# invictus717/MiCo

Measured on AMD Instinct MI355X. Metric: omni-modal samples/sec (ViT-g/14 fwd+bwd), higher is better.
Workload: dtype fp16

## Files before the change

### include/mico_hip.h

```cpp
#ifndef MICO_HIP_H
#define MICO_HIP_H
#include <stdint.h>

#ifdef __cplusplus
extern "C" {
#endif

#define MICO_F16 0
#define MICO_BF16 1
#define MICO_F32 2

#define MICO_OK 0
#define MICO_EINVAL (-22)
#define MICO_ELAUNCH (-5)

int mico_version(void);
const char* mico_last_error_string(void);
int mico_struct_layout(int* out, int n);

#define MICO_ACT_NONE 0
#define MICO_ACT_GELU 1
#define MICO_ACT_GELU_GRAD 2
#define MICO_ACT_GELU_SAVE_DERIV 3
#define MICO_ACT_MUL_AUX 4
// ... 9 lines not shown
    const float* resid;
    const float* pos;
    int pos_rows;
    int remap_group;
    int remap_skip;
    int remap_offset;
    float alpha;
    int accumulate;
    int nseg, kseg;
    int a_seg_off[3], b_seg_off[3];
    const int* row_map;
    int rows_per_map;
    float drop_p;
    unsigned drop_seed;
    int drop_site;
    float* colsum_out;
    void* splitk_ws;
    int64_t splitk_ws_bytes;
    int aux_tiled;
} mico_gemm_epilogue;

int mico_gemm_last_kernel(void);
int64_t mico_gemm_aux_tiled_elems(int64_t M, int64_t N, int64_t K);
int mico_gemm(int ta, int tb, int64_t M, int64_t N, int64_t K,
              const void* A, int64_t lda, const void* B, int64_t ldb,
              void* C, int64_t ldc, int c_dtype,
              const mico_gemm_epilogue* epi, int split_k, int dtype, void* stream);

int mico_quant_mx8(const void* x, int64_t ld, int64_t rows, int cols, void* q, int64_t ldq, void* scales, float pre_scale,
                   int dtype, void* stream);
int mico_gemm_mx8(int64_t M, int64_t N, int64_t K, const void* A, int64_t lda, const void* a_scales, const void* B, int64_t ldb,
                  const void* b_scales, void* C, int64_t ldc, int c_dtype, const mico_gemm_epilogue* epi, int out_dtype, void* stream);

typedef struct mico_ln_fwd_params {
    const void* x;
    int x_dtype;
    int x_normalized;
    const float* gamma;
    const float* beta;
    void* y16;
    float* y32;
    float* mean;
    float* rstd;
    int64_t rows;
    int cols;
    float eps;
// ... 189 lines not shown
```

### mico_amd/_lib.py

```python
import ctypes as C
import os

import torch

_HERE = os.path.dirname(os.path.abspath(__file__))
LIB_PATH = os.environ.get("MICO_HIP_LIB") or os.path.join(_HERE, "libmico_hip.so")

F16, BF16, F32 = 0, 1, 2
ACT_NONE, ACT_GELU, ACT_GELU_GRAD, ACT_GELU_SAVE_DERIV, ACT_MUL_AUX = 0, 1, 2, 3, 4

c_i64, c_int, c_f, c_vp = C.c_int64, C.c_int, C.c_float, C.c_void_p


class GemmEpilogue(C.Structure):
    _fields_ = [
        ("bias", c_vp), ("aux_out", c_vp), ("aux_in", c_vp), ("ldaux", c_i64), ("act", c_int),
        ("row_scale", c_vp), ("rows_per_scale", c_int), ("resid", c_vp), ("pos", c_vp), ("pos_rows", c_int),
        ("remap_group", c_int), ("remap_skip", c_int), ("remap_offset", c_int), ("alpha", c_f), ("accumulate", c_int),
        ("nseg", c_int), ("kseg", c_int), ("a_seg_off", c_int * 3), ("b_seg_off", c_int * 3),
        ("row_map", c_vp), ("rows_per_map", c_int),
        ("drop_p", c_f), ("drop_seed", C.c_uint), ("drop_site", c_int), ("colsum_out", c_vp),
        ("splitk_ws", c_vp), ("splitk_ws_bytes", c_i64), ("aux_tiled", c_int),
    ]

# ... 14 lines not shown
        ("mean", c_vp), ("rstd", c_vp), ("rows", c_i64), ("cols", c_int), ("eps", c_f), ("post_add", c_vp),
        ("post_rows_per_group", c_int), ("post_groups", c_int), ("y16_split", c_int), ("frame_map", c_vp), ("rows_per_frame", c_int),
        ("x_copy", c_vp), ("xhat16", c_vp), ("drop_p", c_f), ("drop_seed", C.c_uint), ("drop_site", c_int), ("valid_cols", c_int),
        ("q8", c_vp), ("ldq", c_i64), ("scales", c_vp),
    ]


class LnBwdParams(C.Structure):
    _fields_ = [
        ("dy", c_vp), ("dy_dtype", c_int), ("dy_scale", c_f), ("x", c_vp), ("x_dtype", c_int), ("x_normalized", c_int), ("gamma", c_vp),
        ("mean", c_vp), ("rstd", c_vp), ("dx_add", c_vp), ("dx32", c_vp), ("dx16", c_vp), ("scale16", c_f), ("dgamma", c_vp),
        ("dbeta", c_vp), ("grad_scale", c_f), ("ws", c_vp), ("rows", c_i64), ("cols", c_int), ("frame_map", c_vp), ("rows_per_frame", c_int),
        ("valid_cols", c_int), ("dx16_dst", c_vp), ("dx16_frame_scale", c_vp), ("dx16_drop_p", c_f), ("dx16_drop_seed", C.c_uint),
        ("dx16_drop_site", c_int),
    ]


PROTOTYPES = {
    "mico_version": [],
    "mico_last_error_string": [],
    "mico_struct_layout": [C.POINTER(c_int), c_int],
    "mico_gemm_last_kernel": [],
    "mico_gemm_aux_tiled_elems": [c_i64, c_i64, c_i64],
    "mico_gemm": [c_int, c_int, c_i64, c_i64, c_i64, c_vp, c_i64, c_vp, c_i64, c_vp, c_i64, c_int,
                  C.POINTER(GemmEpilogue), c_int, c_int, c_vp],
    "mico_quant_mx8": [c_vp, c_i64, c_i64, c_int, c_vp, c_i64, c_vp, c_f, c_int, c_vp],
    "mico_gemm_mx8": [c_i64, c_i64, c_i64, c_vp, c_i64, c_vp, c_vp, c_i64, c_vp, c_vp, c_i64, c_int, C.POINTER(GemmEpilogue), c_int, c_vp],
    "mico_layernorm_fwd": [C.POINTER(LnFwdParams), c_int, c_vp],
    "mico_layernorm_bwd_nblk": [c_i64],
    "mico_layernorm_bwd": [C.POINTER(LnBwdParams), c_int, c_vp],
    "mico_attn_fwd": [c_vp, c_vp, c_vp, c_vp, c_vp, C.POINTER(AttnParams), c_int, c_vp],
    "mico_attn_bwd": [c_vp, c_vp, c_vp, c_vp, c_vp, c_vp, c_vp, c_vp, c_vp, c_vp, C.POINTER(AttnParams), c_int, c_vp],
    "mico_attn_decode_ws_bytes": [c_int, c_int, c_int, c_int, c_int],
    "mico_attn_decode": [c_vp, c_i64, c_vp, c_vp, c_i64, c_i64, c_vp, c_i64, c_vp, c_i64, c_i64, c_int, c_int, c_int, c_int, c_int,
                         c_int, c_f, c_int, c_vp, c_i64, c_int, c_vp],
    "mico_decode_kv_append": [c_vp, c_i64, c_vp, c_i64, c_i64, c_int, c_int, c_int, c_int, c_vp],
    "mico_decode_kv_gather": [c_vp, c_vp, c_vp, c_int, c_int, c_i64, c_i64, c_i64, c_vp],
    "mico_rope": [c_vp, c_i64, c_i64, c_int, c_int, c_int, c_int, c_vp, c_vp, c_int, c_int, c_vp],
    "mico_im2row": [c_vp, c_vp, c_int, c_int, c_int, c_int, c_int, c_int, c_int, c_vp],
    "mico_im2row_keep": [c_vp, c_vp, c_vp, c_int, c_int, c_int, c_int, c_int, c_int, c_int, c_int, c_vp],
    "mico_patch_pos_keep": [c_vp, c_i64, c_vp, c_int, c_int, c_vp, c_vp, c_int, c_int, c_vp],
    "mico_rope_keep": [c_vp, c_i64, c_i64, c_int, c_int, c_int, c_int, c_vp, c_vp, c_vp, c_int, c_vp, c_int, c_int, c_int, c_vp],
    "mico_pos_grad_keep": [c_vp, c_i64, c_vp, c_int, c_int, c_int, c_int, c_vp, c_vp, c_vp],
    "mico_cast_f32_to_16": [c_vp, c_i64, c_vp, c_i64, c_i64, c_int, c_int, c_f, c_int, c_vp],
    "mico_cast_16_to_f32": [c_vp, c_i64, c_vp, c_i64, c_i64, c_int, c_f, c_int, c_int, c_vp],
    "mico_gather_rows_cast": [c_vp, c_i64, c_vp, c_i64, c_i64, c_int, c_int, c_int, c_int, c_vp, c_int, c_f, c_vp, c_int,
# ... 29 lines not shown
    "mico_l2norm_bwd": [c_vp, c_vp, c_vp, c_vp, c_i64, c_int, c_vp],
    "mico_image_preprocess": [c_vp, c_int, c_int, c_int, c_vp, c_int, c_int, c_f, c_f, c_f, c_f, c_f, c_f, c_vp],
    "mico_fbank_windows": [c_vp, c_int, c_int, c_vp, c_int, c_int, c_f, c_f, c_vp, c_vp],
    "mico_adamw_step": [c_vp, c_int, c_vp, c_vp, c_int, c_int, c_f, c_f, c_f, c_f, c_f, c_f, c_f, c_vp],
    "mico_grads_finite": [c_vp, c_int, c_vp, c_vp, c_int, c_int, c_vp, c_vp],
    "mico_comm_unique_id": [c_vp],
    "mico_comm_init": [C.POINTER(c_vp), c_int, c_int, c_vp],
    "mico_comm_destroy": [c_vp],
    "mico_comm_allgather": [c_vp, c_vp, c_vp, c_i64, c_vp],
    "mico_comm_allgather_packed": [c_vp, C.POINTER(c_vp), C.POINTER(c_i64), c_int, c_i64, c_vp, c_vp, c_vp],
    "mico_comm_alltoallv": [c_vp, c_vp, C.POINTER(c_i64), c_vp, C.POINTER(c_i64), c_vp],
    "mico_comm_allreduce_f32": [c_vp, c_vp, c_i64, c_int, c_vp],
    "mico_comm_reduce_scatter_f32": [c_vp, c_vp, c_vp, c_i64, c_int, c_vp],
}
_RESTYPES = {"mico_last_error_string": C.c_char_p, "mico_gemm_aux_tiled_elems": c_i64}

_lib = None


class MicoHipError(RuntimeError):
    pass


ABI_VERSION = 117


def _check_struct_layout(l):
    n = l.mico_struct_layout(None, 0)
    buf = (c_int * n)()
    l.mico_struct_layout(buf, n)
    table, cur = [], []
    for v in buf:
        if v == -1:
            table.append(cur)
            cur = []
        else:
            cur.append(v)
    classes = (GemmEpilogue, AttnParams, LnFwdParams, LnBwdParams)
    if len(table) != len(classes):
        raise MicoHipError(f"mico_struct_layout reports {len(table)} structs, this binding mirrors {len(classes)}")
    for cls, (size, *offs) in zip(classes, table):
        mine = [getattr(cls, name).offset for name, _ in cls._fields_]
        if C.sizeof(cls) != size or mine != offs:
            raise MicoHipError(f"ctypes {cls.__name__} does not match the compiled struct (size {C.sizeof(cls)} vs {size}, offsets {mine} vs {offs})")


def lib():
# ... 38 lines not shown
```

### mico_amd/csrc/gemm.hip

```cpp
#include "common.h"
#include <stdarg.h>
#include <stddef.h>
#include <stdio.h>
#include <algorithm>
#include <type_traits>

#ifndef MICO_W4_DBG
#define MICO_W4_DBG 0
#endif
#ifndef MICO_W4_STAGGER
#define MICO_W4_STAGGER 1
#endif
#ifndef MICO_BIG_MIDBAR
#define MICO_BIG_MIDBAR 2
#endif
#ifndef MICO_SLAB_FIXED
#define MICO_SLAB_FIXED 48
#endif
#ifndef MICO_GEMM_ABLATE
#define MICO_GEMM_ABLATE 0
#endif

#if MICO_GEMM_ABLATE == 7
__device__ unsigned long long g_mico_phase_times[8192 * 8];
// ... 34 lines not shown
#define MICO_MID_PRIO 0
#endif
#ifndef MICO_MID_IL
#define MICO_MID_IL 0
#endif
#ifndef MICO_MID_GROUP_M
#define MICO_MID_GROUP_M 4
#endif

template <int BM_, int BN_, int WM_, int WN_, int BK_, int STAGES_> struct TileCfg {
    static constexpr int BM = BM_, BN = BN_, WM = WM_, WN = WN_, BK = BK_, STAGES = STAGES_;
    static constexpr int WAVES = WM * WN, THREADS = WAVES * 64;
    static constexpr int MT = BM / WM / 16, NT = BN / WN / 16;
    static constexpr int KSTEPS = BK / 32;
    static constexpr int A_BYTES = BM * BK * 2, B_BYTES = BN * BK * 2, STAGE_BYTES = A_BYTES + B_BYTES;
    static constexpr int A_DMA = A_BYTES / 16 / THREADS, B_DMA = B_BYTES / 16 / THREADS;
    static constexpr int LDS_BYTES = STAGES * STAGE_BYTES;
    static_assert(NT == 4, "wave tiles are 64 columns wide");
};
using Big = TileCfg<256, 256, 2, 4, 32, 4>;
using Small = TileCfg<128, 128, 2, 2, 64, 2>;
using Mid = TileCfg<256, 128, 2, 2, 32, 3>;

struct GemmArgs {
    const char* A;
    const char* B;
    char* C;
    int64_t M, N, K, lda, ldb, ldc;
    int ntm, ntn, ntiles, split_k, ktiles, ktiles_per_split;
    int c_dtype;
    int group_m;
    int fast16;
    int tm0;
    int a_wrap;
    int64_t ka_rows, kb_rows;
    mico_gemm_epilogue e;
};

__device__ __forceinline__ int key_kc(int row) { return (row >> 1) & 7; }
__device__ __forceinline__ int key_k32(int row) { return (0x1230 >> (((row >> 2) & 3) * 4)) & 3; }
__device__ __forceinline__ int key_tr(int row) { return ((row & 3) | (((row >> 3) & 1) << 2)) << 1; }

#ifndef MICO_ASM_DMA
#define MICO_ASM_DMA 1
#endif
template <bool ASM>
__device__ __forceinline__ void lds_dma16(__amdgpu_buffer_rsrc_t rs, LDS_AS void* lds_dst, unsigned voff) {
    if constexpr (ASM && MICO_ASM_DMA) {
        unsigned keep;
        const unsigned dst = __builtin_amdgcn_readfirstlane((unsigned)(uintptr_t)lds_dst);
        asm volatile("s_mov_b32 %0, m0\n\ts_mov_b32 m0, %2\n\ts_nop 0\n\tbuffer_load_dwordx4 %1, %3, 0 offen lds\n\ts_mov_b32 m0, %0"
                     : "=&s"(keep) : "v"(voff), "s"(dst), "s"(rs) : "memory");
    } else {
        __builtin_amdgcn_raw_ptr_buffer_load_lds(rs, lds_dst, 16, voff, 0, 0, 0);
    }
}

__device__ __forceinline__ void lds_dma16_soff(__amdgpu_buffer_rsrc_t rs, LDS_AS void* lds_dst, unsigned voff, unsigned soff) {
// ... 2268 lines not shown
#else
#define PC_BARRIER() __builtin_amdgcn_s_barrier()
#endif
#ifndef MICO_PC_MIDBAR
#define MICO_PC_MIDBAR 0
#endif
#if MICO_PC_MIDBAR
#define PC_MIDBAR() PC_BARRIER()
#else
#define PC_MIDBAR() do {} while (0)
#endif
template <typename T, bool TA, bool TB, int BKW>
__global__ __launch_bounds__(Wide<BKW>::THREADS) void gemm_pc_kernel(const GemmArgs g) {
    using CFG = Wide<BKW>;
    constexpr int BM = CFG::BM, BN = CFG::BN, BK = CFG::BK, MT = CFG::MT, PTH = CFG::PTHREADS, ND = CFG::NDMA;
    constexpr int RING = CFG::STAGES * CFG::STAGE_BYTES;
    __shared__ __attribute__((aligned(16))) char smem[CFG::LDS_BYTES];
    LDS_AS char* lds = (LDS_AS char*)smem;
    const int lane = threadIdx.x & 63;
    const int wave = __builtin_amdgcn_readfirstlane(threadIdx.x >> 6);

    int bid;
    int ks;
    {
        const int W = g.ntiles * g.split_k, b0 = blockIdx.x;
        const int nx = 8, q = W / nx, r = W % nx, x = b0 % nx, o = b0 / nx;
        const int lin = (x < r ? x * (q + 1) : r * (q + 1) + (x - r) * q) + o;
        ks = lin / g.ntiles;
        bid = lin - ks * g.ntiles;
    }
    int tile_m, tile_n;
    {
        const int gsz = GROUP_M * g.ntn;
        const int grp = bid / gsz;
        const int first = grp * GROUP_M;
        const int gm = min(g.ntm - first, GROUP_M);
        const int in = bid - grp * gsz;
        tile_m = first + in % gm;
        tile_n = in / gm;
    }
    const int64_t m0 = (int64_t)tile_m * BM, n0 = (int64_t)tile_n * BN;
    const int kt0 = ks * g.ktiles_per_split;
    const int kt1 = min(g.ktiles, kt0 + g.ktiles_per_split);
    const int T_ = kt1 - kt0;

    if (wave >= CFG::CWAVES) {
        const int pw = wave - CFG::CWAVES;
        const int64_t lda_b = g.lda * 2, ldb_b = g.ldb * 2;
        const char* a_base = TA ? g.A + m0 * 2 : g.A + m0 * lda_b;
        const char* b_base = TB ? g.B + n0 * 2 : g.B + n0 * ldb_b;
        int64_t a_bytes = TA ? g.ka_rows * lda_b - m0 * 2 : (g.M - m0) * lda_b;
        int64_t b_bytes = TB ? g.kb_rows * ldb_b - n0 * 2 : (g.N - n0) * ldb_b;
        if (a_bytes > 0xFFFFFF00ll) a_bytes = 0xFFFFFF00ll;
        if (b_bytes > 0xFFFFFF00ll) b_bytes = 0xFFFFFF00ll;
        __amdgpu_buffer_rsrc_t rsa = __builtin_amdgcn_make_buffer_rsrc((void*)a_base, 0, (int)a_bytes, 0x00020000);
        __amdgpu_buffer_rsrc_t rsb = __builtin_amdgcn_make_buffer_rsrc((void*)b_base, 0, (int)b_bytes, 0x00020000);
        const int64_t a_crem = min(g.M - m0, (int64_t)BM), b_crem = g.N - n0;
        unsigned voa[ND], vob[ND];
        dma_offsets<TA, 256, PTH, BK, ND>(voa, pw, lane, lda_b, a_crem);
        dma_offsets<TB, 256, PTH, BK, ND>(vob, pw, lane, ldb_b, b_crem);
        constexpr int NA = TA ? ND : ND - ND / 4;
        constexpr int PTI = NA + ND;
        const int nseg = g.e.nseg, kseg = g.e.kseg;
        const bool ktail = (g.K % BK) != 0;
        auto stage = [&](int kt, int bo, int part = 3) {
            const int k0 = kt * BK;
            int ka = k0, kb = k0;
            int64_t kda = g.K, kdb = g.K;
            if (nseg > 0) {
                const int sg = k0 / kseg, kin = k0 - sg * kseg;
                ka = g.e.a_seg_off[sg] + kin;
                kb = g.e.b_seg_off[sg] + kin;
                kda = g.e.a_seg_off[sg] + kseg;
                kdb = g.e.b_seg_off[sg] + kseg;
            }
            if ((MICO_GEMM_ABLATE == 1 || MICO_GEMM_ABLATE == 10 || MICO_GEMM_ABLATE == 11) && kt >= kt0 + 3) return;
            if (ktail && kt == g.ktiles - 1) {
                if (part & 1) stage_tile<TA, 256, PTH, BK>(rsa, lds + bo, pw, lane, lda_b, ka, kda, a_crem);
                if (part & 2) stage_tile<TB, 256, PTH, BK>(rsb, lds + bo + CFG::A_BYTES, pw, lane, ldb_b, kb, kdb, b_crem);
                return;
            }
            const unsigned koa = TA ? (unsigned)((int64_t)ka * lda_b) : (unsigned)(ka * 2);
            const unsigned kob = TB ? (unsigned)((int64_t)kb * ldb_b) : (unsigned)(kb * 2);
            if (part & 1) dma_issue<PTH, ND, NA>(rsa, lds + bo, pw, voa, koa);
            if (part & 2) dma_issue<PTH, ND, ND>(rsb, lds + bo + CFG::A_BYTES, pw, vob, kob);
        };
        constexpr int AHEAD = CFG::STAGES - 1;
        for (int i = 0; i < AHEAD && i < T_; ++i) stage(kt0 + i, i * CFG::STAGE_BYTES);
        const bool do_colsum = TA && TB && g.e.colsum_out != nullptr;
        const int cs_ntn = g.ntn;
        int cs_phase = do_colsum ? (tile_n + cs_ntn - kt0 % cs_ntn) % cs_ntn : 0;
        const int pid = pw * 64 + lane, lc = pid & 31, rg = pid >> 5;
        const unsigned cbase = (unsigned)(uintptr_t)lds + (unsigned)rg * 512u;
        const unsigned cx_even = cbase + (unsigned)((lc ^ ((rg & 3) << 1)) << 4), cx_odd = cbase + (unsigned)((lc ^ (((rg & 3) | 4) << 1)) << 4);
        float cs[8] = {0.f, 0.f, 0.f, 0.f, 0.f, 0.f, 0.f, 0.f};
        int bo = 0;
        for (int t = 0; t < T_; ++t) {
            asm volatile("" : "+s"(bo));
            const int ahead = T_ - 1 - t;
            if (AHEAD >= 3 && ahead >= 2) asm volatile("s_waitcnt vmcnt(%0)" ::"n"(2 * PTI) : "memory");
            else if (AHEAD >= 3 && ahead == 1) asm volatile("s_waitcnt vmcnt(%0)" ::"n"(PTI) : "memory");
            else asm volatile("s_waitcnt vmcnt(0)" ::: "memory");
            PC_BARRIER();
            __builtin_amdgcn_sched_barrier(0);
            const bool refill = t + AHEAD < T_;
            const int rbo = (bo + AHEAD * CFG::STAGE_BYTES) & (RING - 1);
            if (refill) stage(kt0 + t + AHEAD, rbo, CFG::KSTEPS == 1 ? 1 : 3);
            __builtin_amdgcn_sched_barrier(0);
            if constexpr (TA && TB) {
                if (do_colsum) {
                    if (cs_phase == 0) {
                        tile_colsum32<T>(cs, cx_even + (unsigned)bo, cx_odd + (unsigned)bo, rg);
                        if constexpr (BK == 64) tile_colsum32<T>(cs, cx_even + (unsigned)bo + 32u * 512u, cx_odd + (unsigned)bo + 32u * 512u, rg);
                        cs_phase = cs_ntn;
                    }
                    --cs_phase;
                }
            }
            __builtin_amdgcn_sched_barrier(0);
#pragma unroll
            for (int r = 0; r < 2 * CFG::KSTEPS - 1; ++r) {
                PC_MIDBAR();
                __builtin_amdgcn_sched_barrier(0);
            }
            if (CFG::KSTEPS == 1 && refill) stage(kt0 + t + AHEAD, rbo, 2);
            __builtin_amdgcn_sched_barrier(0);
            bo = (bo + CFG::STAGE_BYTES) & (RING - 1);
        }
        PC_BARRIER();
        if (do_colsum) {
#pragma unroll
            for (int k = 0; k < 8; ++k) {
                const float v = cs[k] + __shfl_xor(cs[k], 32, 64);
                const int col = lc * 8 + k;
                if (lane < 32 && col < BM && m0 + col < g.M) unsafeAtomicAdd(g.e.colsum_out + m0 + col, v * g.e.alpha);
            }
        }
        return;
    }

    const int wm = wave >> 2, wn = wave & 3;
    f32x4 acc[MT][4];
#pragma unroll
    for (int i = 0; i < MT; ++i)
#pragma unroll
        for (int j = 0; j < 4; ++j) acc[i][j] = (f32x4){0.f, 0.f, 0.f, 0.f};
    const FragBase ab = frag_base<TA, 256, BK>(wm * 64, lane), ab2 = frag_base<TA, 256, BK>(128 + wm * 32, lane);
    const FragBase bb = frag_base<TB, 256, BK>(wn * 64, lane);
    s16x8 fa[MT], fb[4];
    auto read_k = [&](int bo, int kk) {
        if (MICO_GEMM_ABLATE == 2 && g.K > 0) {
#pragma unroll
            for (int i = 0; i < MT; ++i) asm volatile("" : "+v"(fa[i]));
#pragma unroll
            for (int j = 0; j < 4; ++j) asm volatile("" : "+v"(fb[j]));
            return;
        }
        LDS_AS const char* ta = lds + bo;
// ... 46 lines not shown
        for (int t = 0; t < T_; ++t) {
            asm volatile("" : "+s"(bo));
            head();
            if (t > 0) mma_k();
            bar();
            read_k(bo, 0);
            if constexpr (CFG::KSTEPS == 2) {
                bar();
                mma_k();
                bar();
                read_k(bo, 1);
            }
            __builtin_amdgcn_sched_barrier(0);
            bo = (bo + CFG::STAGE_BYTES) & (RING - 1);
        }
        if (T_ > 0) {
            asm volatile("s_waitcnt lgkmcnt(0)" ::: "memory");
            mma_k();
        }
    }
    asm volatile("s_waitcnt lgkmcnt(0)" ::: "memory");
    PC_BARRIER();
    __builtin_amdgcn_sched_barrier(0);
#pragma unroll
    for (int hb = 0; hb < 3; ++hb) {
        const int64_t mrow = m0 + (hb < 2 ? wm * 64 + hb * 32 : 128 + wm * 32);
        if (g.split_k > 1 && g.e.splitk_ws == nullptr) gemm_epilogue_atomic<2>(g, &acc[hb * 2], mrow, n0 + wn * 64, lane);
        else if (g.split_k > 1) {
            GemmArgs gp = g;
            gp.C = (char*)g.e.splitk_ws + (int64_t)ks * g.M * g.N * 4;
            gp.ldc = g.N;
            gp.c_dtype = MICO_F32;
            gp.e.alpha = 1.f;
            gp.e.accumulate = 0;
            gemm_epilogue_block<T, 2, ACT_LEAN>(gp, &acc[hb * 2], lds + wave * 8192, mrow, n0 + wn * 64, lane);
        } else gemm_epilogue_block<T, 2, ACT_LEAN>(g, &acc[hb * 2], lds + wave * 8192, mrow, n0 + wn * 64, lane);
    }
}


#ifdef MICO_GEMM_W4
template <int DEEP> struct W4C {
    static constexpr int BM = 256, BN = 256, BK = DEEP ? 32 : 64, STAGES = DEEP ? 4 : 2, THREADS = 256, MT = 8;
    static constexpr int A_BYTES = 256 * BK * 2, STAGE_BYTES = 2 * A_BYTES, LDS_BYTES = STAGES * STAGE_BYTES;
    static constexpr int NDMA = A_BYTES / 16 / THREADS;
};
using W4 = W4C<0>;

template <typename T, bool TA, bool TB, int ACT, int P1, int DEEP>
__global__ __launch_bounds__(W4::THREADS) __attribute__((amdgpu_waves_per_eu(1, 1))) void gemm_w4_kernel(const GemmArgs g) {
    using W4 = W4C<DEEP>;
    constexpr int BM = W4::BM, BN = W4::BN, BK = W4::BK, THREADS = W4::THREADS, ND = W4::NDMA;
    constexpr int STAGE = W4::STAGE_BYTES;
    __shared__ __attribute__((aligned(16))) char smem[W4::LDS_BYTES];
    LDS_AS char* lds = (LDS_AS char*)smem;
    const int lane = threadIdx.x & 63;
    const int wave = __builtin_amdgcn_readfirstlane(threadIdx.x >> 6);
    const int wm = wave >> 1, wn = wave & 1;
    const int wrow = wm * 128, wcol = wn * 128;
// ... 217 lines not shown
#pragma unroll
        for (int c = 0; c < 2; ++c)
#pragma unroll
            for (int h = 0; h < 2; ++h) gemm_epilogue_atomic(g, &acc[c][h * 4], m0 + wrow + h * 64, n0 + wcol + c * 64, lane);
    } else {
        asm volatile("s_waitcnt vmcnt(0) lgkmcnt(0)" ::: "memory");
        __syncthreads();
#pragma unroll
        for (int c = 0; c < 2; ++c)
#pragma unroll
            for (int h = 0; h < 2; ++h)
                gemm_epilogue_block<T, 4, ACT>(g, &acc[c][h * 4], lds + wave * 16384, m0 + wrow + h * 64, n0 + wcol + c * 64, lane);
    }
}

#endif

#ifndef MICO_PC_BK
#define MICO_PC_BK 32
#endif
constexpr int pc_bk(int, int) { return MICO_PC_BK; }

__global__ __launch_bounds__(256) void splitk_reduce_kernel(const float* __restrict__ ws, int nsplit, int64_t M, int64_t N, float* __restrict__ C,
                                                            int64_t ldc, float alpha) {
    const int64_t n4 = N / 4, total = M * n4, slab = M * N;
    for (int64_t i = (int64_t)blockIdx.x * 256 + threadIdx.x; i < total; i += (int64_t)gridDim.x * 256) {
        const int64_t m = i / n4, n = (i - m * n4) * 4;
        f32x4 acc = *(const f32x4*)(ws + m * N + n);
        for (int s = 1; s < nsplit; ++s) acc += *(const f32x4*)(ws + s * slab + m * N + n);
        f32x4* cp = (f32x4*)(C + m * ldc + n);
        *cp = *cp + acc * alpha;
    }
}

bool resid_epilogue(const GemmArgs& g) {
#ifdef MICO_NO_RESID_EPI
    return false;
#else
    return g.e.act == MICO_ACT_NONE && !g.e.aux_out && !g.e.aux_in && g.e.drop_p == 0.f && !g.e.pos && !g.e.remap_group && g.e.resid != nullptr &&
           g.c_dtype == MICO_F32 && !g.e.accumulate && g.split_k == 1 && g.e.alpha == 1.f;
#endif
}

template <typename T>
void launch_pc(int ta, int tb, const GemmArgs& g, hipStream_t st) {
    const dim3 grid(g.ntiles * g.split_k), block(Wide<32>::THREADS);
    if (ta && tb) MICO_LAUNCH((gemm_pc_kernel<T, true, true, MICO_PC_BK>), grid, block, 0, st, g);
#ifdef MICO_GEMM_PC_ALL
    else if (!ta && !tb) MICO_LAUNCH((gemm_pc_kernel<T, false, false, 32>), grid, block, 0, st, g);
    else if (!ta && tb) MICO_LAUNCH((gemm_pc_kernel<T, false, true, 32>), grid, block, 0, st, g);
    else MICO_LAUNCH((gemm_pc_kernel<T, true, false, 32>), grid, block, 0, st, g);
#endif
// ... 144 lines not shown

}

thread_local char g_mico_err[256] = "";

int mico_set_err(int code, const char* fmt, ...) {
    va_list ap;
    va_start(ap, fmt);
    vsnprintf(g_mico_err, sizeof(g_mico_err), fmt, ap);
    va_end(ap);
    return code;
}

thread_local int g_mico_last_gemm_kernel = 0;
#ifdef MICO_GEMM_VARIANTS
static int g_mico_gemm_variant = 0;
static int g_mico_mid_group = 0;
extern "C" int mico_gemm_set_variant(int v) { const int old = g_mico_gemm_variant + 100 * g_mico_mid_group; g_mico_gemm_variant = v % 100; g_mico_mid_group = v / 100; return old; }
#else
static constexpr int g_mico_gemm_variant = 0;
static constexpr int g_mico_mid_group = 0;
#endif
extern "C" int mico_gemm_last_kernel(void) { return g_mico_last_gemm_kernel; }
extern "C" int mico_version(void) { return 117; }
extern "C" const char* mico_last_error_string(void) { return g_mico_err; }

extern "C" int mico_struct_layout(int* out, int n) {
#define OFF(S, F) (int)offsetof(S, F)
    const int t[] = {
        (int)sizeof(mico_gemm_epilogue),
        OFF(mico_gemm_epilogue, bias), OFF(mico_gemm_epilogue, aux_out), OFF(mico_gemm_epilogue, aux_in), OFF(mico_gemm_epilogue, ldaux),
        OFF(mico_gemm_epilogue, act), OFF(mico_gemm_epilogue, row_scale), OFF(mico_gemm_epilogue, rows_per_scale), OFF(mico_gemm_epilogue, resid),
        OFF(mico_gemm_epilogue, pos), OFF(mico_gemm_epilogue, pos_rows), OFF(mico_gemm_epilogue, remap_group), OFF(mico_gemm_epilogue, remap_skip),
        OFF(mico_gemm_epilogue, remap_offset), OFF(mico_gemm_epilogue, alpha), OFF(mico_gemm_epilogue, accumulate), OFF(mico_gemm_epilogue, nseg),
        OFF(mico_gemm_epilogue, kseg), OFF(mico_gemm_epilogue, a_seg_off), OFF(mico_gemm_epilogue, b_seg_off), OFF(mico_gemm_epilogue, row_map),
        OFF(mico_gemm_epilogue, rows_per_map), OFF(mico_gemm_epilogue, drop_p), OFF(mico_gemm_epilogue, drop_seed), OFF(mico_gemm_epilogue, drop_site),
        OFF(mico_gemm_epilogue, colsum_out), OFF(mico_gemm_epilogue, splitk_ws), OFF(mico_gemm_epilogue, splitk_ws_bytes),
        OFF(mico_gemm_epilogue, aux_tiled),
        -1,
        (int)sizeof(mico_attn_params),
        OFF(mico_attn_params, B), OFF(mico_attn_params, H), OFF(mico_attn_params, Sq), OFF(mico_attn_params, Sk), OFF(mico_attn_params, hd),
        OFF(mico_attn_params, q_bs), OFF(mico_attn_params, q_rs), OFF(mico_attn_params, k_bs), OFF(mico_attn_params, k_rs), OFF(mico_attn_params, v_bs),
        OFF(mico_attn_params, v_rs), OFF(mico_attn_params, o_bs), OFF(mico_attn_params, o_rs), OFF(mico_attn_params, scale), OFF(mico_attn_params, mask),
        OFF(mico_attn_params, mask_mode), OFF(mico_attn_params, drop_p), OFF(mico_attn_params, drop_seed), OFF(mico_attn_params, drop_site),
        OFF(mico_attn_params, kv_batch_mod), OFF(mico_attn_params, batch0), OFF(mico_attn_params, dkv_accumulate),
        OFF(mico_attn_params, kv_index),
        -1,
// ... 85 lines not shown
                       else DISPATCH_T16(out_dtype, MICO_LAUNCH((gemm_mx8_kernel<T, ACTV>), grid, block, 0, st, a)); } while (0)
    const bool persist = MICO_P8_PERSIST && p8mx && g.fast16 && N % 8 == 0 && g.ntiles > 256 && g.ktiles >= 2 && !g.e.aux_in && g_mico_gemm_variant != 17;
    if (persist && g.e.act == MICO_ACT_GELU_SAVE_DERIV) DISPATCH_T16(out_dtype, MICO_LAUNCH((gemm_p8pmx_kernel<T, MICO_ACT_GELU_SAVE_DERIV>), dim3(256), block, 0, st, a));
    else if (persist && lean) DISPATCH_T16(out_dtype, MICO_LAUNCH((gemm_p8pmx_kernel<T, ACT_LEAN>), dim3(256), block, 0, st, a));
    else if (g.e.act == MICO_ACT_GELU_SAVE_DERIV) MX8(MICO_ACT_GELU_SAVE_DERIV);
    else if (g.e.act == MICO_ACT_MUL_AUX) MX8(MICO_ACT_MUL_AUX);
    else if (lean) MX8(ACT_LEAN);
    else DISPATCH_T16(out_dtype, MICO_LAUNCH((gemm_mx8_kernel<T, 0>), grid, block, 0, st, a));
#undef MX8
    MICO_LAUNCH_CHECK();
    return MICO_OK;
}

extern "C" int64_t mico_gemm_aux_tiled_elems(int64_t M, int64_t N, int64_t K) {
    static const bool no_wrap = getenv("MICO_P8_NOWRAP") != nullptr;
    if (!MICO_P8_PERSIST || !MICO_P8_DEFAULT || g_mico_gemm_variant != 0 || no_wrap) return 0;
    if (M <= 0 || N <= 0 || K <= 0 || N % 256 != 0 || K % 64 != 0 || K < 128) return 0;
    const int64_t tiles = ((M + 255) / 256) * (N / 256);
    if (tiles <= 256 || tiles >= 0x7FFFFFFFll) return 0;
    if (256 * N * 2 >= 0x7FFFFFFFll || 256 * (2 * K) * 2 + 2 * K * 2 >= 0x7FFFFF00ll || (K + 64) * N * 2 >= 0x7FFFFF00ll) return 0;
    return ((M + 255) / 256) * 256 * N;
}

extern "C" int mico_gemm(int ta, int tb, int64_t M, int64_t N, int64_t K, const void* A, int64_t lda, const void* B,
                         int64_t ldb, void* C, int64_t ldc, int c_dtype, const mico_gemm_epilogue* epi, int split_k,
                         int dtype, void* stream) {
    MICO_CHECK(dtype_ok(dtype), "mico_gemm: dtype must be MICO_F16 or MICO_BF16");
    MICO_CHECK(A && B && C, "mico_gemm: null operand");
    MICO_CHECK(M > 0 && N > 0 && K > 0, "mico_gemm: empty problem M=%lld N=%lld K=%lld", (long long)M, (long long)N, (long long)K);
    MICO_CHECK(lda % 8 == 0 && ldb % 8 == 0, "mico_gemm: lda/ldb must be multiples of 8 elements (got %lld, %lld)", (long long)lda, (long long)ldb);
    MICO_CHECK(N % 4 == 0 && ldc % 4 == 0, "mico_gemm: N and ldc must be multiples of 4 (got %lld, %lld)", (long long)N, (long long)ldc);
    if (c_dtype != MICO_F32) MICO_CHECK(ldc % 8 == 0 && ((uintptr_t)C & 15) == 0, "mico_gemm: a 16-bit C needs ldc %% 8 == 0 and a 16-byte aligned base (16-byte stores)");
    if (epi && (epi->aux_out || epi->aux_in)) MICO_CHECK(epi->ldaux % 8 == 0, "mico_gemm: ldaux must be a multiple of 8");
    const bool segs = epi && epi->nseg > 0;
    if (!ta) MICO_CHECK(K % 8 == 0 && (segs || lda >= K), "mico_gemm: A[M,K] needs K %% 8 == 0 and lda >= K");
    else MICO_CHECK(lda >= M, "mico_gemm: A^T[K,M] needs lda >= M");
    if (!tb) MICO_CHECK(K % 8 == 0 && (segs || ldb >= K), "mico_gemm: B[N,K] needs K %% 8 == 0 and ldb >= K");
    else MICO_CHECK(ldb >= N, "mico_gemm: B^T[K,N] needs ldb >= N");
    MICO_CHECK(c_dtype == MICO_F32 || c_dtype == dtype, "mico_gemm: c_dtype must be MICO_F32 or dtype");
    MICO_CHECK(256 * lda * 2 < 0x7FFFFFFFll && 256 * ldb * 2 < 0x7FFFFFFFll, "mico_gemm: leading dimension too large");
    if (ta) MICO_CHECK(K * lda * 2 <= 0xFFFFFF00ll, "mico_gemm: A^T[K,M] spans %lld bytes (K * lda * 2); reduction-major operands are limited to 4 GiB per launch", (long long)(K * lda * 2));
    if (tb) MICO_CHECK(K * ldb * 2 <= 0xFFFFFF00ll, "mico_gemm: B^T[K,N] spans %lld bytes (K * ldb * 2); reduction-major operands are limited to 4 GiB per launch", (long long)(K * ldb * 2));
    GemmArgs g;
    g.A = (const char*)A; g.B = (const char*)B; g.C = (char*)C;
    g.M = M; g.N = N; g.K = K; g.lda = lda; g.ldb = ldb; g.ldc = ldc;
    g.c_dtype = c_dtype;
// ... 23 lines not shown
#else
    const bool w4_built = false;
#endif
    const bool w4 = w4_built && big && g_mico_gemm_variant >= 2 && (ta || K % 64 == 0) && (tb || K % 64 == 0) && a_ext < 0x7FFFFF00ll && b_ext < 0x7FFFFF00ll;
    if (w4) pc = false;
    const bool no_split = split_k == 1 || (split_k <= 0 && !(c_dtype == MICO_F32 && g.e.accumulate));
    const bool mid = big && !pc && !w4 && !ta && no_split &&
                     (g_mico_gemm_variant == 5 || (g_mico_gemm_variant == 6 && K <= 2048));
    const bool mid_default = (g_mico_gemm_variant == 0 || g_mico_gemm_variant == 11 || g_mico_gemm_variant == 16) && M >= 8192 &&
                             (g.e.act == MICO_ACT_GELU_SAVE_DERIV || (g.e.resid != nullptr && c_dtype == MICO_F32 && K <= 2048));
    static const bool no_wrap = getenv("MICO_P8_NOWRAP") != nullptr;
    const bool wrap_ok = !no_wrap && g.e.nseg == 2 && !ta && !tb && g.e.kseg % 64 == 0 && g.e.a_seg_off[0] == 0 && g.e.a_seg_off[1] == 0 &&
                         g.e.b_seg_off[0] == 0 && g.e.b_seg_off[1] == g.e.kseg;
    const bool p8_ok = big && !pc && !w4 && !ta && no_split && N % 4 == 0 && K % 64 == 0 && (g.e.nseg == 0 || wrap_ok) &&
                       256 * lda * 2 + K * 2 < 0x7FFFFF00ll && (tb ? (K + 64) * ldb * 2 : 256 * ldb * 2 + K * 2) < 0x7FFFFF00ll;
    const bool p8 = p8_ok && (g_mico_gemm_variant == 10 || g_mico_gemm_variant == 13 || g_mico_gemm_variant == 14 || g_mico_gemm_variant == 15 || (g_mico_gemm_variant == 11 && !mid_default) ||
                              ((g_mico_gemm_variant == 0 || g_mico_gemm_variant == 16) && MICO_P8_DEFAULT));
    const bool mid64 = big && !pc && !w4 && !p8 && !ta && no_split && N % 4 == 0 && K % 64 == 0 && (g.e.nseg == 0 || g.e.kseg % 64 == 0) &&
                       (g_mico_gemm_variant == 8 || (g_mico_gemm_variant == 9 && K <= 2048) || mid_default);
    const int BM = pc ? Wide<32>::BM : (big ? 256 : 128), BN = (mid || mid64) ? 128 : (big ? 256 : 128);
    const int slots = big && !mid && !mid64 ? 256 : 512;
    g.ntm = (int)((M + BM - 1) / BM); g.ntn = (int)((N + BN - 1) / BN);
    g.ntiles = g.ntm * g.ntn;
    const bool deep = g_mico_gemm_variant == 3;
    const int BKc = w4 ? (deep ? 32 : 64) : pc ? pc_bk(ta, tb) : p8 ? P8C::BK : mid64 ? Mid64::BK : mid ? Mid::BK : (big ? Big::BK : Small::BK);
    g.ktiles = (int)((K + BKc - 1) / BKc);
    if (split_k <= 0) {
        if (!(c_dtype == MICO_F32 && g.e.accumulate)) split_k = 1;
        else if (!big && g.ntiles <= 512 && g.e.splitk_ws && g.e.splitk_ws_bytes >= 2 * M * N * 4 && N % 4 == 0)
            split_k = small_slab_split(g.ntiles, g.ktiles, (double)M * N, (int)std::min<int64_t>(32, g.e.splitk_ws_bytes / (M * N * 4)));
        else if (!big && g.ntiles <= 512) split_k = small_acc_split(g.ntiles, g.ktiles);
        else if (pc && g.e.splitk_ws && g.e.splitk_ws_bytes >= 2 * M * N * 4) {
            const int max_s = (int)std::min<int64_t>(32, g.e.splitk_ws_bytes / (M * N * 4));
            split_k = auto_split(g.ntiles, g.ktiles, slots, 1024 / BKc, MICO_SLAB_FIXED, max_s, (int)(M * N / 590000) + 8);
        }
        else split_k = auto_split(g.ntiles, g.ktiles, slots, big ? 1024 / BKc : 16, big ? 5440 / BKc : 12);
    }
    if (split_k > g.ktiles) split_k = g.ktiles;
    g.ktiles_per_split = (g.ktiles + split_k - 1) / split_k;
    split_k = (g.ktiles + g.ktiles_per_split - 1) / g.ktiles_per_split;
    g.split_k = split_k;
    if (!((pc || !big) && split_k > 1 && g.e.splitk_ws && g.e.splitk_ws_bytes >= (int64_t)split_k * M * N * 4 && N % 4 == 0 &&
          ((uintptr_t)C & 15) == 0 && ((uintptr_t)g.e.splitk_ws & 15) == 0))
        g.e.splitk_ws = nullptr;
    g.ka_rows = g.kb_rows = K;
    g.group_m = g_mico_mid_group > 0 ? g_mico_mid_group : MICO_MID_GROUP_M;
    if (g.e.nseg > 0) {
        MICO_CHECK(g.e.nseg <= 3 && g.e.kseg > 0 && g.e.kseg % 64 == 0 && (int64_t)g.e.nseg * g.e.kseg == K,
                   "mico_gemm: k-segments need nseg <= 3, kseg %% 64 == 0 and nseg * kseg == K");
        g.ka_rows = g.kb_rows = 0;
        for (int i = 0; i < g.e.nseg; ++i) {
            MICO_CHECK(g.e.a_seg_off[i] % 8 == 0 && g.e.b_seg_off[i] % 8 == 0 && g.e.a_seg_off[i] >= 0 && g.e.b_seg_off[i] >= 0, "mico_gemm: bad segment offset");
            if (g.e.a_seg_off[i] + g.e.kseg > g.ka_rows) g.ka_rows = g.e.a_seg_off[i] + g.e.kseg;
            if (g.e.b_seg_off[i] + g.e.kseg > g.kb_rows) g.kb_rows = g.e.b_seg_off[i] + g.e.kseg;
        }
    }
    if (g.split_k > 1) {
        MICO_CHECK(c_dtype == MICO_F32 && g.e.accumulate, "mico_gemm: split_k > 1 needs fp32 accumulate output");
        MICO_CHECK(!g.e.bias && !g.e.aux_out && g.e.act == MICO_ACT_NONE && !g.e.row_scale && !g.e.resid && !g.e.pos && !g.e.remap_group && !g.e.row_map && g.e.drop_p == 0.f,
                   "mico_gemm: split_k > 1 supports only the alpha-scaled accumulate epilogue");
    }
    if (g.e.act == MICO_ACT_GELU_GRAD || g.e.act == MICO_ACT_MUL_AUX) MICO_CHECK(g.e.aux_in != nullptr, "mico_gemm: GELU_GRAD / MUL_AUX need aux_in");
    if (g.e.act == MICO_ACT_GELU_GRAD && g.e.aux_out) MICO_CHECK(c_dtype != MICO_F32 && g.e.aux_out != g.e.aux_in, "mico_gemm: GELU_GRAD with aux_out (= gelu(aux_in)) needs a 16-bit C and a buffer of its own");
    MICO_CHECK(g.e.act >= MICO_ACT_NONE && g.e.act <= MICO_ACT_MUL_AUX, "mico_gemm: unknown act %d", g.e.act);
    if (g.e.act == MICO_ACT_GELU_SAVE_DERIV) MICO_CHECK(!ta && !tb && g.e.aux_out && c_dtype != MICO_F32, "mico_gemm: GELU_SAVE_DERIV is the forward epilogue (ta = tb = 0, aux_out, 16-bit C)");
    if (g.e.act == MICO_ACT_MUL_AUX) MICO_CHECK(!ta && tb, "mico_gemm: MUL_AUX is the dX epilogue (ta = 0, tb = 1)");
    if (g.e.act == MICO_ACT_GELU_SAVE_DERIV || g.e.act == MICO_ACT_MUL_AUX)
// ... 51 lines not shown
            g2.tm0 = ntm1;
            g2.ntm = g.ntm - ntm1;
            g2.ntn = (int)((N + 127) / 128);
            g2.ntiles = g2.ntm * g2.ntn;
            g.ntm = ntm1;
            g.ntiles = g.ntm * g.ntn;
            DISPATCH_T16(dtype, (launch_p8<T>(tb, g, st, g_mico_gemm_variant != 16)));
            DISPATCH_T16(dtype, (launch_mid<T>(tb, g2, st)));
        } else DISPATCH_T16(dtype, (launch_p8<T>(tb, g, st, g_mico_gemm_variant != 16)));
    }
    else if (mid64) { g_mico_last_gemm_kernel = 7; DISPATCH_T16(dtype, (launch_mid<T>(tb, g, st))); }
#ifdef MICO_GEMM_VARIANTS
    else if (mid) { g_mico_last_gemm_kernel = 6; DISPATCH_T16(dtype, (launch<T, Mid>(ta, tb, g, st))); }
#endif
    else if (big) {
        bool done = false;
        if (g.split_k == 1 && g.ntiles >= 512 && g.e.nseg == 0 && K % 32 == 0 && g_mico_gemm_variant != 4) DISPATCH_T16(dtype, (done = launch_persist<T>(ta, tb, g, st)));
        if (done) g_mico_last_gemm_kernel = 5;
        else DISPATCH_T16(dtype, (launch<T, Big>(ta, tb, g, st)));
    }
    else DISPATCH_T16(dtype, (launch<T, Small>(ta, tb, g, st)));
    if (g.e.splitk_ws) {
        MICO_LAUNCH_CHECK();
        const int64_t total = M * (N / 4);
        MICO_LAUNCH(splitk_reduce_kernel, dim3((unsigned)std::min<int64_t>((total + 255) / 256, 4096)), dim3(256), 0, st, (const float*)g.e.splitk_ws,
                    g.split_k, M, N, (float*)C, ldc, g.e.alpha);
    }
    MICO_LAUNCH_CHECK();
    return MICO_OK;
}
```

Measured before the change: 42.92.

## Mix swapped-orientation tiles in weight-gradient GEMM to cut tile count

For the transposed-A/transposed-B producer-consumer weight-gradient GEMM, a planner splits the output into two regions. One uses the normal 192x256 tiling and the other computes the transposed product with operands swapped, picking the cut that minimizes total tiles and wave quantization. Both regions write to the split-k slab workspace, and a new transposing reduce kernel folds the swapped region back into C. This adds per-block part selection, an extra reduction launch and workspace traffic even when split_k is 1, and it is on by default unless MICO_PC_MIXED=0.

```diff
diff --git a/include/mico_hip.h b/include/mico_hip.h
--- a/include/mico_hip.h
+++ b/include/mico_hip.h
@@ -55,6 +55,7 @@
 
 int mico_gemm_last_kernel(void);
 int64_t mico_gemm_aux_tiled_elems(int64_t M, int64_t N, int64_t K);
+int mico_gemm_pc_plan(int64_t M, int64_t N, int mixed, int* tiles, int cap);
 int mico_gemm(int ta, int tb, int64_t M, int64_t N, int64_t K,
               const void* A, int64_t lda, const void* B, int64_t ldb,
               void* C, int64_t ldc, int c_dtype,
diff --git a/mico_amd/_lib.py b/mico_amd/_lib.py
--- a/mico_amd/_lib.py
+++ b/mico_amd/_lib.py
@@ -60,6 +60,7 @@
     "mico_struct_layout": [C.POINTER(c_int), c_int],
     "mico_gemm_last_kernel": [],
     "mico_gemm_aux_tiled_elems": [c_i64, c_i64, c_i64],
+    "mico_gemm_pc_plan": [c_i64, c_i64, c_int, C.POINTER(c_int), c_int],
     "mico_gemm": [c_int, c_int, c_i64, c_i64, c_i64, c_vp, c_i64, c_vp, c_i64, c_vp, c_i64, c_int,
                   C.POINTER(GemmEpilogue), c_int, c_int, c_vp],
     "mico_quant_mx8": [c_vp, c_i64, c_i64, c_int, c_vp, c_i64, c_vp, c_f, c_int, c_vp],
@@ -135,7 +136,7 @@
     pass
 
 
-ABI_VERSION = 117
+ABI_VERSION = 118
 
 
 def _check_struct_layout(l):
diff --git a/mico_amd/csrc/gemm.hip b/mico_amd/csrc/gemm.hip
--- a/mico_amd/csrc/gemm.hip
+++ b/mico_amd/csrc/gemm.hip
@@ -80,6 +80,53 @@
 using Small = TileCfg<128, 128, 2, 2, 64, 2>;
 using Mid = TileCfg<256, 128, 2, 2, 32, 3>;
 
+struct PcPlan {
+    int mix;
+    int nplain;
+    int ntm[2], ntn[2];
+    int64_t roff[2], R[2];
+    int64_t coff[2], Cn[2];
+    int64_t wsoff[2];
+};
+
+__host__ __device__ __forceinline__ void pc_tile_of(int ntm, int ntn, int bid, int& tile_m, int& tile_n) {
+    const int gsz = GROUP_M * ntn;
+    const int grp = bid / gsz;
+    const int first = grp * GROUP_M;
+    const int gm = (ntm - first < GROUP_M) ? ntm - first : GROUP_M;
+    const int in = bid - grp * gsz;
+    tile_m = first + in % gm;
+    tile_n = in / gm;
+}
+
+inline PcPlan pc_plan(int64_t M, int64_t N, bool mixed) {
+    auto cd = [](int64_t a, int64_t b) { return (int)((a + b - 1) / b); };
+    int best = cd(M, 192) * cd(N, 256), mix = 0;
+    int64_t cut = 0;
+    if (mixed && M % 4 == 0 && N % 4 == 0) {
+        for (int64_t c = 256; c < N; c += 256) {
+            const int n = cd(M, 192) * (int)(c / 256) + cd(N - c, 192) * cd(M, 256);
+            if (n < best) { best = n; mix = 1; cut = c; }
+        }
+        for (int64_t c = 256; c < M; c += 256) {
+            const int n = (int)(c / 256) * cd(N, 192) + cd(M - c, 192) * cd(N, 256);
+            if (n < best) { best = n; mix = 2; cut = c; }
+        }
+    }
+    PcPlan p{};
+    p.mix = mix;
+    p.roff[0] = mix == 2 ? cut : 0; p.R[0] = M - p.roff[0];
+    p.coff[0] = 0;                  p.Cn[0] = mix == 1 ? cut : N;
+    if (mix == 1)      { p.roff[1] = cut; p.R[1] = N - cut; p.coff[1] = 0; p.Cn[1] = M; }
+    else if (mix == 2) { p.roff[1] = 0;   p.R[1] = N;       p.coff[1] = 0; p.Cn[1] = cut; }
+    for (int i = 0; i < 2; ++i) { p.ntm[i] = cd(p.R[i], 192); p.ntn[i] = cd(p.Cn[i], 256); }
+    p.nplain = p.ntm[0] * p.ntn[0];
+    p.wsoff[0] = 0;
+    p.wsoff[1] = p.R[0] * p.Cn[0];
+    return p;
+}
+inline int pc_plan_tiles(const PcPlan& p) { return p.nplain + p.ntm[1] * p.ntn[1]; }
+
 struct GemmArgs {
     const char* A;
     const char* B;
@@ -92,6 +139,7 @@
     int tm0;
     int a_wrap;
     int64_t ka_rows, kb_rows;
+    PcPlan pc;
     mico_gemm_epilogue e;
 };
 
@@ -2406,23 +2454,27 @@
 
     int bid;
     int ks;
+    int part = 0;
     {
         const int W = g.ntiles * g.split_k, b0 = blockIdx.x;
         const int nx = 8, q = W / nx, r = W % nx, x = b0 % nx, o = b0 / nx;
-        const int lin = (x < r ? x * (q + 1) : r * (q + 1) + (x - r) * q) + o;
-        ks = lin / g.ntiles;
-        bid = lin - ks * g.ntiles;
-    }
+        int lin = (x < r ? x * (q + 1) : r * (q + 1) + (x - r) * q) + o;
+        int np = g.ntiles;
+        if constexpr (TA && TB) {
+            const int w0 = g.pc.nplain * g.split_k;
+            part = lin >= w0;
+            np = part ? g.ntiles - g.pc.nplain : g.pc.nplain;
+            if (part) lin -= w0;
+        }
+        ks = lin / np;
+        bid = lin - ks * np;
+    }
+    const bool sw = part != 0;
+    auto part_rows = [&](bool s_) -> int64_t { return !(TA && TB) ? g.M : s_ ? g.pc.R[1] : g.pc.R[0]; };
+    auto part_cols = [&](bool s_) -> int64_t { return !(TA && TB) ? g.N : s_ ? g.pc.Cn[1] : g.pc.Cn[0]; };
+    auto opaque = [](int v) { v = __builtin_amdgcn_readfirstlane(v); asm volatile("" : "+s"(v)); return v; };
     int tile_m, tile_n;
-    {
-        const int gsz = GROUP_M * g.ntn;
-        const int grp = bid / gsz;
-        const int first = grp * GROUP_M;
-        const int gm = min(g.ntm - first, GROUP_M);
-        const int in = bid - grp * gsz;
-        tile_m = first + in % gm;
-        tile_n = in / gm;
-    }
+    pc_tile_of(!(TA && TB) ? g.ntm : sw ? g.pc.ntm[1] : g.pc.ntm[0], !(TA && TB) ? g.ntn : sw ? g.pc.ntn[1] : g.pc.ntn[0], bid, tile_m, tile_n);
     const int64_t m0 = (int64_t)tile_m * BM, n0 = (int64_t)tile_n * BN;
     const int kt0 = ks * g.ktiles_per_split;
     const int kt1 = min(g.ktiles, kt0 + g.ktiles_per_split);
@@ -2430,16 +2482,22 @@
 
     if (wave >= CFG::CWAVES) {
         const int pw = wave - CFG::CWAVES;
-        const int64_t lda_b = g.lda * 2, ldb_b = g.ldb * 2;
-        const char* a_base = TA ? g.A + m0 * 2 : g.A + m0 * lda_b;
-        const char* b_base = TB ? g.B + n0 * 2 : g.B + n0 * ldb_b;
-        int64_t a_bytes = TA ? g.ka_rows * lda_b - m0 * 2 : (g.M - m0) * lda_b;
-        int64_t b_bytes = TB ? g.kb_rows * ldb_b - n0 * 2 : (g.N - n0) * ldb_b;
+        const int64_t pR = part_rows(sw), pC = part_cols(sw);
+        const char* const opa = sw ? g.B : g.A;
+        const char* const opb = sw ? g.A : g.B;
+        const int64_t lda_b = (sw ? g.ldb : g.lda) * 2, ldb_b = (sw ? g.lda : g.ldb) * 2;
+        const int64_t a_rows = sw ? g.kb_rows : g.ka_rows, b_rows = sw ? g.ka_rows : g.kb_rows;
+        const int64_t ac0 = ((TA && TB) ? (sw ? g.pc.roff[1] : g.pc.roff[0]) : 0) + m0;
+        const int64_t bc0 = ((TA && TB) ? (sw ? g.pc.coff[1] : g.pc.coff[0]) : 0) + n0;
+        const char* a_base = TA ? opa + ac0 * 2 : opa + ac0 * lda_b;
+        const char* b_base = TB ? opb + bc0 * 2 : opb + bc0 * ldb_b;
+        int64_t a_bytes = TA ? a_rows * lda_b - ac0 * 2 : (g.M - m0) * lda_b;
+        int64_t b_bytes = TB ? b_rows * ldb_b - bc0 * 2 : (g.N - n0) * ldb_b;
         if (a_bytes > 0xFFFFFF00ll) a_bytes = 0xFFFFFF00ll;
         if (b_bytes > 0xFFFFFF00ll) b_bytes = 0xFFFFFF00ll;
         __amdgpu_buffer_rsrc_t rsa = __builtin_amdgcn_make_buffer_rsrc((void*)a_base, 0, (int)a_bytes, 0x00020000);
         __amdgpu_buffer_rsrc_t rsb = __builtin_amdgcn_make_buffer_rsrc((void*)b_base, 0, (int)b_bytes, 0x00020000);
-        const int64_t a_crem = min(g.M - m0, (int64_t)BM), b_crem = g.N - n0;
+        const int64_t a_crem = min(pR - m0, (int64_t)BM), b_crem = pC - n0;
         unsigned voa[ND], vob[ND];
         dma_offsets<TA, 256, PTH, BK, ND>(voa, pw, lane, lda_b, a_crem);
         dma_offsets<TB, 256, PTH, BK, ND>(vob, pw, lane, ldb_b, b_crem);
@@ -2471,11 +2529,12 @@
         };
         constexpr int AHEAD = CFG::STAGES - 1;
         for (int i = 0; i < AHEAD && i < T_; ++i) stage(kt0 + i, i * CFG::STAGE_BYTES);
-        const bool do_colsum = TA && TB && g.e.colsum_out != nullptr;
-        const int cs_ntn = g.ntn;
-        int cs_phase = do_colsum ? (tile_n + cs_ntn - kt0 % cs_ntn) % cs_ntn : 0;
+        const bool do_colsum = TA && TB && g.e.colsum_out != nullptr && !(sw && g.pc.mix == 1);
+        const int cs_ntn = !(TA && TB) ? g.ntn : sw ? g.pc.ntm[1] : g.pc.ntn[0];
+        const int cs_idx = sw ? tile_m : tile_n;
+        int cs_phase = do_colsum ? (cs_idx + cs_ntn - kt0 % cs_ntn) % cs_ntn : 0;
         const int pid = pw * 64 + lane, lc = pid & 31, rg = pid >> 5;
-        const unsigned cbase = (unsigned)(uintptr_t)lds + (unsigned)rg * 512u;
+        const unsigned cbase = (unsigned)(uintptr_t)lds + (unsigned)rg * 512u + (sw ? (unsigned)CFG::A_BYTES : 0u);
         const unsigned cx_even = cbase + (unsigned)((lc ^ ((rg & 3) << 1)) << 4), cx_odd = cbase + (unsigned)((lc ^ (((rg & 3) | 4) << 1)) << 4);
         float cs[8] = {0.f, 0.f, 0.f, 0.f, 0.f, 0.f, 0.f, 0.f};
         int bo = 0;
@@ -2513,11 +2572,14 @@
         }
         PC_BARRIER();
         if (do_colsum) {
+            const bool s2 = (TA && TB) && opaque(part) != 0;
+            const int64_t cs_c0 = !(TA && TB) ? m0 : s2 ? g.pc.coff[1] + n0 : g.pc.roff[0] + m0;
+            const int cs_cols = (int)min(s2 ? part_cols(true) - n0 : part_rows(false) - m0, (int64_t)(s2 ? BN : BM));
 #pragma unroll
             for (int k = 0; k < 8; ++k) {
                 const float v = cs[k] + __shfl_xor(cs[k], 32, 64);
                 const int col = lc * 8 + k;
-                if (lane < 32 && col < BM && m0 + col < g.M) unsafeAtomicAdd(g.e.colsum_out + m0 + col, v * g.e.alpha);
+                if (lane < 32 && col < cs_cols) unsafeAtomicAdd(g.e.colsum_out + cs_c0 + col, v * g.e.alpha);
             }
         }
         return;
@@ -2610,19 +2672,24 @@
     asm volatile("s_waitcnt lgkmcnt(0)" ::: "memory");
     PC_BARRIER();
     __builtin_amdgcn_sched_barrier(0);
+    const bool swe = (TA && TB) && opaque(part) != 0;
+    const int64_t pR = part_rows(swe), pC = part_cols(swe);
+    const bool slab = g.e.splitk_ws != nullptr;
+    GemmArgs gp = g;
+    if (slab) {
+        gp.C = (char*)g.e.splitk_ws + ((int64_t)ks * g.M * g.N + ((TA && TB) ? (swe ? g.pc.wsoff[1] : g.pc.wsoff[0]) : 0)) * 4;
+        gp.M = pR;
+        gp.N = pC;
+        gp.ldc = pC;
+        gp.c_dtype = MICO_F32;
+        gp.e.alpha = g.split_k > 1 ? 1.f : g.e.alpha;
+        gp.e.accumulate = 0;
+    }
 #pragma unroll
     for (int hb = 0; hb < 3; ++hb) {
         const int64_t mrow = m0 + (hb < 2 ? wm * 64 + hb * 32 : 128 + wm * 32);
-        if (g.split_k > 1 && g.e.splitk_ws == nullptr) gemm_epilogue_atomic<2>(g, &acc[hb * 2], mrow, n0 + wn * 64, lane);
-        else if (g.split_k > 1) {
-            GemmArgs gp = g;
-            gp.C = (char*)g.e.splitk_ws + (int64_t)ks * g.M * g.N * 4;
-            gp.ldc = g.N;
-            gp.c_dtype = MICO_F32;
-            gp.e.alpha = 1.f;
-            gp.e.accumulate = 0;
-            gemm_epilogue_block<T, 2, ACT_LEAN>(gp, &acc[hb * 2], lds + wave * 8192, mrow, n0 + wn * 64, lane);
-        } else gemm_epilogue_block<T, 2, ACT_LEAN>(g, &acc[hb * 2], lds + wave * 8192, mrow, n0 + wn * 64, lane);
+        if (g.split_k > 1 && !slab) gemm_epilogue_atomic<2>(g, &acc[hb * 2], mrow, n0 + wn * 64, lane);
+        else gemm_epilogue_block<T, 2, ACT_LEAN>(gp, &acc[hb * 2], lds + wave * 8192, mrow, n0 + wn * 64, lane);
     }
 }
 
@@ -2886,12 +2953,42 @@
 constexpr int pc_bk(int, int) { return MICO_PC_BK; }
 
 __global__ __launch_bounds__(256) void splitk_reduce_kernel(const float* __restrict__ ws, int nsplit, int64_t M, int64_t N, float* __restrict__ C,
-                                                            int64_t ldc, float alpha) {
-    const int64_t n4 = N / 4, total = M * n4, slab = M * N;
+                                                            int64_t ldc, float alpha, int64_t slab) {
+    const int64_t n4 = N / 4, total = M * n4;
     for (int64_t i = (int64_t)blockIdx.x * 256 + threadIdx.x; i < total; i += (int64_t)gridDim.x * 256) {
         const int64_t m = i / n4, n = (i - m * n4) * 4;
         f32x4 acc = *(const f32x4*)(ws + m * N + n);
         for (int s = 1; s < nsplit; ++s) acc += *(const f32x4*)(ws + s * slab + m * N + n);
+        f32x4* cp = (f32x4*)(C + m * ldc + n);
+        *cp = *cp + acc * alpha;
+    }
+}
+
+__global__ __launch_bounds__(256) void splitk_reduce_t_kernel(const float* __restrict__ wt, int nsplit, int64_t Mt, int64_t Nt, float* __restrict__ C,
+                                                              int64_t ldc, float alpha, int64_t slab) {
+    __shared__ float t[64][65];
+    const int64_t tm = (Mt + 63) / 64;
+    const int64_t m0 = (blockIdx.x % tm) * 64, n0 = (blockIdx.x / tm) * 64;
+    const int r = threadIdx.x >> 4, c4 = (threadIdx.x & 15) * 4;
+#pragma unroll
+    for (int i = 0; i < 4; ++i) {
+        const int64_t n = n0 + r + i * 16, m = m0 + c4;
+        f32x4 acc = {0.f, 0.f, 0.f, 0.f};
+        if (n < Nt && m < Mt) {
+            acc = *(const f32x4*)(wt + n * Mt + m);
+            for (int s = 1; s < nsplit; ++s) acc += *(const f32x4*)(wt + s * slab + n * Mt + m);
+        }
+#pragma unroll
+        for (int k = 0; k < 4; ++k) t[r + i * 16][c4 + k] = acc[k];
+    }
+    __syncthreads();
+#pragma unroll
+    for (int i = 0; i < 4; ++i) {
+        const int64_t m = m0 + r + i * 16, n = n0 + c4;
+        if (m >= Mt || n >= Nt) continue;
+        f32x4 acc;
+#pragma unroll
+        for (int k = 0; k < 4; ++k) acc[k] = t[c4 + k][r + i * 16];
         f32x4* cp = (f32x4*)(C + m * ldc + n);
         *cp = *cp + acc * alpha;
     }
@@ -3082,7 +3179,7 @@
 static constexpr int g_mico_mid_group = 0;
 #endif
 extern "C" int mico_gemm_last_kernel(void) { return g_mico_last_gemm_kernel; }
-extern "C" int mico_version(void) { return 117; }
+extern "C" int mico_version(void) { return 118; }
 extern "C" const char* mico_last_error_string(void) { return g_mico_err; }
 
 extern "C" int mico_struct_layout(int* out, int n) {
@@ -3214,6 +3311,24 @@
     return ((M + 255) / 256) * 256 * N;
 }
 
+extern "C" int mico_gemm_pc_plan(int64_t M, int64_t N, int mixed, int* tiles, int cap) {
+    MICO_CHECK(M > 0 && N > 0 && M < 0x7FFFFFFFll && N < 0x7FFFFFFFll, "mico_gemm_pc_plan: bad problem M=%lld N=%lld", (long long)M, (long long)N);
+    const PcPlan p = pc_plan(M, N, mixed != 0);
+    const int n = pc_plan_tiles(p);
+    for (int i = 0; i < n && i < cap && tiles; ++i) {
+        const int part = i >= p.nplain, bid = part ? i - p.nplain : i;
+        int tm, tn;
+        pc_tile_of(p.ntm[part], p.ntn[part], bid, tm, tn);
+        const int64_t r0 = (int64_t)tm * Wide<32>::BM, c0 = (int64_t)tn * Wide<32>::BN;
+        const int64_t rr = std::min<int64_t>(Wide<32>::BM, p.R[part] - r0), cc = std::min<int64_t>(Wide<32>::BN, p.Cn[part] - c0);
+        int* t = tiles + 5 * i;
+        t[0] = part;
+        if (!part) { t[1] = (int)(p.roff[0] + r0); t[2] = (int)(p.coff[0] + c0); t[3] = (int)rr; t[4] = (int)cc; }
+        else       { t[1] = (int)(p.coff[1] + c0); t[2] = (int)(p.roff[1] + r0); t[3] = (int)cc; t[4] = (int)rr; }
+    }
+    return n;
+}
+
 extern "C" int mico_gemm(int ta, int tb, int64_t M, int64_t N, int64_t K, const void* A, int64_t lda, const void* B,
                          int64_t ldb, void* C, int64_t ldc, int c_dtype, const mico_gemm_epilogue* epi, int split_k,
                          int dtype, void* stream) {
@@ -3283,6 +3398,16 @@
     const int slots = big && !mid && !mid64 ? 256 : 512;
     g.ntm = (int)((M + BM - 1) / BM); g.ntn = (int)((N + BN - 1) / BN);
     g.ntiles = g.ntm * g.ntn;
+    g.pc = PcPlan{};
+    if (pc && ta && tb) {
+        const char* const sw_env = getenv("MICO_PC_MIXED");
+        const bool mixed_on = !(sw_env && atoi(sw_env) == 0);
+        const int64_t slabs = split_k > 0 ? split_k : 2;
+        const bool mixed = mixed_on && c_dtype == MICO_F32 && g.e.accumulate && g.e.nseg == 0 && !g.e.bias && !g.e.row_scale && !g.e.resid && !g.e.row_map && g.e.splitk_ws &&
+                           g.e.splitk_ws_bytes >= slabs * M * N * 4 && ((uintptr_t)C & 15) == 0 && ((uintptr_t)g.e.splitk_ws & 15) == 0;
+        g.pc = pc_plan(M, N, mixed);
+        g.ntiles = pc_plan_tiles(g.pc);
+    }
     const bool deep = g_mico_gemm_variant == 3;
     const int BKc = w4 ? (deep ? 32 : 64) : pc ? pc_bk(ta, tb) : p8 ? P8C::BK : mid64 ? Mid64::BK : mid ? Mid::BK : (big ? Big::BK : Small::BK);
     g.ktiles = (int)((K + BKc - 1) / BKc);
@@ -3301,9 +3426,10 @@
     g.ktiles_per_split = (g.ktiles + split_k - 1) / split_k;
     split_k = (g.ktiles + g.ktiles_per_split - 1) / g.ktiles_per_split;
     g.split_k = split_k;
-    if (!((pc || !big) && split_k > 1 && g.e.splitk_ws && g.e.splitk_ws_bytes >= (int64_t)split_k * M * N * 4 && N % 4 == 0 &&
+    if (!((pc || !big) && (split_k > 1 || g.pc.mix) && g.e.splitk_ws && g.e.splitk_ws_bytes >= (int64_t)split_k * M * N * 4 && N % 4 == 0 &&
           ((uintptr_t)C & 15) == 0 && ((uintptr_t)g.e.splitk_ws & 15) == 0))
         g.e.splitk_ws = nullptr;
+    MICO_CHECK(!g.pc.mix || g.e.splitk_ws, "mico_gemm: internal - a mixed weight-gradient tile list without its slab scratch");
     g.ka_rows = g.kb_rows = K;
     g.group_m = g_mico_mid_group > 0 ? g_mico_mid_group : MICO_MID_GROUP_M;
     if (g.e.nseg > 0) {
@@ -3401,9 +3527,20 @@
     else DISPATCH_T16(dtype, (launch<T, Small>(ta, tb, g, st)));
     if (g.e.splitk_ws) {
         MICO_LAUNCH_CHECK();
-        const int64_t total = M * (N / 4);
-        MICO_LAUNCH(splitk_reduce_kernel, dim3((unsigned)std::min<int64_t>((total + 255) / 256, 4096)), dim3(256), 0, st, (const float*)g.e.splitk_ws,
-                    g.split_k, M, N, (float*)C, ldc, g.e.alpha);
+        const float* ws = (const float*)g.e.splitk_ws;
+        const float ralpha = g.split_k > 1 ? g.e.alpha : 1.f;
+        const int64_t pM = g.pc.mix ? g.pc.R[0] : M, pN = g.pc.mix ? g.pc.Cn[0] : N, slab = M * N;
+        const int64_t total = pM * (pN / 4);
+        float* Cp = (float*)C + (g.pc.mix ? g.pc.roff[0] * ldc : 0);
+        if (total > 0)
+            MICO_LAUNCH(splitk_reduce_kernel, dim3((unsigned)std::min<int64_t>((total + 255) / 256, 4096)), dim3(256), 0, st, ws, g.split_k, pM, pN, Cp, ldc,
+                        ralpha, slab);
+        if (g.pc.mix) {
+            MICO_LAUNCH_CHECK();
+            const int64_t Mt = g.pc.Cn[1], Nt = g.pc.R[1];
+            MICO_LAUNCH(splitk_reduce_t_kernel, dim3((unsigned)(((Mt + 63) / 64) * ((Nt + 63) / 64))), dim3(256), 0, st, ws + g.pc.wsoff[1], g.split_k, Mt, Nt,
+                        (float*)C + g.pc.coff[1] * ldc + g.pc.roff[1], ldc, ralpha, slab);
+        }
     }
     MICO_LAUNCH_CHECK();
     return MICO_OK;
```

New measurement: 42.73. Within noise of the previous version (-0.4%).
